# vrgamegirl19/comfyui-vrgamedevgirl

Hardware: NVIDIA H100
Metric: megapixels/sec (grain+LUT+colormatch+sharpen chain) at 4K (higher is better)
Workload: dtype f32

## Files before the change

### comfyui-vrgamedevgirl_b200/csrc/vrgdg_abi.cu

```cuda
#include "../../include/vrgdg_b200.h"
#include "vrgdg_kernels.cuh"
#include <cmath>
#include "vrgdg_adjust.cuh"
#include "vrgdg_resize.cuh"
#include "vrgdg_lanczos.cuh"
#include "vrgdg_temporal.cuh"
#include "vrgdg_histmatch.cuh"
#include <atomic>
#include <stdarg.h>
#include <stdio.h>
#include <stdlib.h>
#include <string.h>

namespace vrgdg {
static std::atomic<int64_t> g_launches{0};
void count_launch() { g_launches.fetch_add(1, std::memory_order_relaxed); }
}

using namespace vrgdg;

namespace {

thread_local char t_err[512] = "";
thread_local const char* t_tile_path = "none";
// ... 26 lines not shown
  }
  if (cached_major != 9 || cached_minor != 0)
    return fail(VRGDG_E_UNSUPPORTED, "libvrgdg_b200 holds sm_90a code only; device %d has compute capability %d.%d", dev, cached_major,
                cached_minor);
  ctx.stream = reinterpret_cast<cudaStream_t>(stream);
  ctx.sms = cached_sms;
  return VRGDG_OK;
}

int check_frames(const void* in, const void* out, int B, int H, int W, int dtype, const char* who) {
  if (!dtype_ok(dtype)) return fail(VRGDG_E_INVALID, "%s: unknown dtype %d", who, dtype);
  if (B < 0 || H < 0 || W < 0) return fail(VRGDG_E_INVALID, "%s: negative shape [%d,%d,%d]", who, B, H, W);
  if ((int64_t)H * W >= (int64_t)1 << 31) return fail(VRGDG_E_UNSUPPORTED, "%s: frame of %d x %d pixels exceeds 2^31", who, H, W);
  if ((int64_t)B * H * W == 0) return VRGDG_OK;
  if (!in || !out) return fail(VRGDG_E_INVALID, "%s: null frame pointer", who);
  size_t es = elem_size(dtype);
  if ((reinterpret_cast<uintptr_t>(in) % es) || (reinterpret_cast<uintptr_t>(out) % es))
    return fail(VRGDG_E_ALIGN, "%s: frame pointer not aligned to its element size", who);
  return VRGDG_OK;
}

#define DISPATCH_DTYPE(dtype, CALL)                                        \
  ((dtype) == VRGDG_F32 ? CALL(float) : ((dtype) == VRGDG_F16 ? CALL(__half) : ((dtype) == VRGDG_BF16 ? CALL(__nv_bfloat16) : CALL(uint8_t))))

typedef CUresult (*encode_fn_t)(CUtensorMap*, CUtensorMapDataType, cuuint32_t, void*, const cuuint64_t*,
                                const cuuint64_t*, const cuuint32_t*, const cuuint32_t*, CUtensorMapInterleave,
                                CUtensorMapSwizzle, CUtensorMapL2promotion, CUtensorMapFloatOOBfill);

encode_fn_t get_encode() {
  static encode_fn_t fn = []() -> encode_fn_t {
    void* p = nullptr;
    cudaDriverEntryPointQueryResult qr;
    if (cudaGetDriverEntryPoint("cuTensorMapEncodeTiled", &p, cudaEnableDefault, &qr) != cudaSuccess ||
        qr != cudaDriverEntryPointSuccess)
      return nullptr;
    return reinterpret_cast<encode_fn_t>(p);
  }();
  return fn;
}

bool build_tmap(CUtensorMap* map, const void* in, int B, int H, int RW, int dtype, int box_x, int box_y) {
  const size_t es = elem_size(dtype);
  if (getenv("VRGDG_NO_TMA")) return false;
  if ((reinterpret_cast<uintptr_t>(in) & 15u) || ((size_t)RW * es) % 16 != 0) return false;
  if (RW < box_x || H < box_y) return false;
  encode_fn_t enc = get_encode();
  if (!enc) return false;
  CUtensorMapDataType dt = dtype == VRGDG_F32 ? CU_TENSOR_MAP_DATA_TYPE_FLOAT32
                         : dtype == VRGDG_F16 ? CU_TENSOR_MAP_DATA_TYPE_FLOAT16
                         : dtype == VRGDG_BF16 ? CU_TENSOR_MAP_DATA_TYPE_BFLOAT16 : CU_TENSOR_MAP_DATA_TYPE_UINT8;
  cuuint64_t dims[3] = {(cuuint64_t)RW, (cuuint64_t)H, (cuuint64_t)B};
  cuuint64_t strides[2] = {(cuuint64_t)RW * es, (cuuint64_t)RW * es * (cuuint64_t)H};
  cuuint32_t box[3] = {(cuuint32_t)box_x, (cuuint32_t)box_y, 1u};
  cuuint32_t estr[3] = {1u, 1u, 1u};
  CUresult r = enc(map, dt, 3, const_cast<void*>(in), dims, strides, box, estr, CU_TENSOR_MAP_INTERLEAVE_NONE,
                   CU_TENSOR_MAP_SWIZZLE_NONE, CU_TENSOR_MAP_L2_PROMOTION_L2_128B, CU_TENSOR_MAP_FLOAT_OOB_FILL_NONE);
  return r == CUDA_SUCCESS;
}

size_t lut_cells_floats(int S) { return (size_t)S * S * S * LUT_CELL_FLOATS; }

void fill_lut(LutParams& L, const float* lut, int S, const float* dmin, const float* dspan, float blend, float omb) {
  L.lut = lut; L.S = S; L.smax = (float)(S - 1);
  L.lutp = lut + lut_cells_floats(S);
  for (int i = 0; i < 3; ++i) { L.dmin[i] = dmin[i]; L.dspan[i] = dspan[i]; }
  L.blend = blend; L.one_minus_blend = omb;
  L.unit_domain = (dmin[0] == 0.f && dmin[1] == 0.f && dmin[2] == 0.f && dspan[0] == 1.f && dspan[1] == 1.f && dspan[2] == 1.f) ? 1 : 0;
}

void zero_point(PointParams& P, int B, int H, int W) {
  memset(&P, 0, sizeof(P));
  P.B = B; P.H = H; P.W = W; P.hw = (int64_t)H * W;
}

int run_tile(const void* in, void* out, int B, int H, int W, int dtype, TileParams& Q, int mask, bool exact, const LaunchCtx& ctx) {
  if (in == out) return fail(VRGDG_E_INVALID, "tile kernels cannot run in place (in == out)");
  Q.B = B; Q.H = H; Q.W = W; Q.RW = 3 * W;
  int bx = 0, by = 0;
#define GEO(T) (tile_geometry<T>(H, Q.RW, Q.tiles_x, Q.tiles_y, bx, by), 0)
  (void)DISPATCH_DTYPE(dtype, GEO);
#undef GEO
  Q.total_tiles = (int64_t)B * Q.tiles_x * Q.tiles_y;
  if (Q.total_tiles >= ((int64_t)1 << 31)) return fail(VRGDG_E_UNSUPPORTED, "batch of %d frames has too many tiles for one launch; split it", B);
  CUtensorMap map;
  bool tma = build_tmap(&map, in, B, H, Q.RW, dtype, bx, by);
  Q.use_tma = tma ? 1 : 0;
  const size_t es = elem_size(dtype);
  Q.vec_store = (((size_t)Q.RW * es) % 16 == 0 && (reinterpret_cast<uintptr_t>(out) & 15u) == 0) ? 1 : 0;
  t_tile_path = tma ? "tma" : "generic";
#define TL(T) launch_tile<T>(tma ? &map : nullptr, in, out, Q, mask, exact, ctx)
  cudaError_t e = DISPATCH_DTYPE(dtype, TL);
#undef TL
  if (e != cudaSuccess) return fail_cuda(e, "k_tile launch");
  return VRGDG_OK;
}

int check_lut(const float* lut, int S, const float* dmin, const float* dspan, const char* who) {
  if (!lut || !dmin || !dspan) return fail(VRGDG_E_INVALID, "%s: null LUT / domain pointer", who);
  if (S < 2 || S > 256) return fail(VRGDG_E_INVALID, "%s: LUT size %d outside [2,256]", who, S);
  if (reinterpret_cast<uintptr_t>(lut) & 31u) return fail(VRGDG_E_ALIGN, "%s: packed LUT must be 32-byte aligned", who);
  return VRGDG_OK;
}

}

extern "C" {

int vrgdg_version(void) { return VRGDG_ABI_VERSION; }
const char* vrgdg_last_error(void) { return t_err; }
int64_t vrgdg_launch_count(void) { return g_launches.load(); }
const char* vrgdg_last_tile_path(void) { return t_tile_path; }

int vrgdg_device_info(int* sm_count, int* cc_major, int* cc_minor) {
  int dev = 0;
  cudaError_t e = cudaGetDevice(&dev);
  if (e != cudaSuccess) return fail_cuda(e, "cudaGetDevice");
  int v = 0;
  if (sm_count) { if ((e = cudaDeviceGetAttribute(&v, cudaDevAttrMultiProcessorCount, dev)) != cudaSuccess) return fail_cuda(e, "attr"); *sm_count = v; }
  if (cc_major) { if ((e = cudaDeviceGetAttribute(&v, cudaDevAttrComputeCapabilityMajor, dev)) != cudaSuccess) return fail_cuda(e, "attr"); *cc_major = v; }
  if (cc_minor) { if ((e = cudaDeviceGetAttribute(&v, cudaDevAttrComputeCapabilityMinor, dev)) != cudaSuccess) return fail_cuda(e, "attr"); *cc_minor = v; }
  return VRGDG_OK;
}

int64_t vrgdg_lut3d_packed_bytes(int lut_size) {
  if (lut_size < 2 || lut_size > 256) return 0;
  return (int64_t)lut_cells_floats(lut_size) * 2 * 4;
}

int vrgdg_lut3d_pack(const float* lut, float* packed, int lut_size, void* stream) {
  if (!lut || !packed) return fail(VRGDG_E_INVALID, "vrgdg_lut3d_pack: null pointer");
  if (lut_size < 2 || lut_size > 256) return fail(VRGDG_E_INVALID, "vrgdg_lut3d_pack: LUT size %d outside [2,256]", lut_size);
  if (reinterpret_cast<uintptr_t>(packed) & 31u) return fail(VRGDG_E_ALIGN, "vrgdg_lut3d_pack: packed buffer must be 32-byte aligned");
  LaunchCtx ctx;
  int rc = get_ctx(stream, ctx);
  if (rc) return rc;
  const int n = lut_size * lut_size * lut_size;
  k_lut_pack<<<(n + 255) / 256, 256, 0, ctx.stream>>>(lut, packed, lut_size);
  count_launch();
  k_lutp_pack<<<(n + 255) / 256, 256, 0, ctx.stream>>>(lut, packed + lut_cells_floats(lut_size), lut_size);
  count_launch();
  cudaError_t e = cudaGetLastError();
  if (e != cudaSuccess) return fail_cuda(e, "vrgdg_lut3d_pack");
  return VRGDG_OK;
}

int vrgdg_lut3d_apply(const void* in, void* out, int64_t npix, int channels, int dtype, const float* lut, int lut_size,
                      const float* dmin_host, const float* dspan_host, float blend, float one_minus_blend, void* stream) {
  if (!dtype_ok(dtype)) return fail(VRGDG_E_INVALID, "vrgdg_lut3d_apply: unknown dtype %d", dtype);
  if (channels != 3 && channels != 4) return fail(VRGDG_E_INVALID, "vrgdg_lut3d_apply: channels must be 3 or 4, got %d", channels);
  if (npix < 0) return fail(VRGDG_E_INVALID, "vrgdg_lut3d_apply: negative pixel count");
  if (!(blend > 0.0f) || blend > 1.0f) return fail(VRGDG_E_INVALID, "vrgdg_lut3d_apply: blend %g outside (0,1]", blend);
  int rc = check_lut(lut, lut_size, dmin_host, dspan_host, "vrgdg_lut3d_apply");
  if (rc) return rc;
  if (npix == 0) return VRGDG_OK;
  if (!in || !out) return fail(VRGDG_E_INVALID, "vrgdg_lut3d_apply: null frame pointer");
  LaunchCtx ctx;
  if ((rc = get_ctx(stream, ctx))) return rc;
  LutParams L;
  fill_lut(L, lut, lut_size, dmin_host, dspan_host, blend, one_minus_blend);
  cudaError_t e;
  if (channels == 4 && dtype == VRGDG_U8BGR) return fail(VRGDG_E_UNSUPPORTED, "vrgdg_lut3d_apply: 4-channel uint8 frames are not supported");
  if (channels == 4) {
#define LR(T) launch_lut_rgba<T>(in, out, npix, L, ctx)
    e = DISPATCH_DTYPE(dtype, LR);
#undef LR
  } else {
    const int64_t chunk = (int64_t)1 << 30;
    e = cudaSuccess;
    for (int64_t p0 = 0; p0 < npix && e == cudaSuccess; p0 += chunk) {
      int64_t n = npix - p0 < chunk ? npix - p0 : chunk;
      PointParams P;
      zero_point(P, 1, 1, (int)n);
      P.lut = L;
// ... 670 lines not shown
```

### comfyui-vrgamedevgirl_b200/csrc/vrgdg_inst.cuh

```cuda
#pragma once
#include "vrgdg_kernels.cuh"
#include <algorithm>
#include "vrgdg_adjust.cuh"
#include "vrgdg_resize.cuh"
#include "vrgdg_temporal.cuh"
#include "vrgdg_histmatch.cuh"
#include <string.h>
#include <stdlib.h>

namespace vrgdg {

static inline bool aligned16(const void* p) { return (reinterpret_cast<uintptr_t>(p) & 15u) == 0; }

template <typename K>
static int occupancy_of(K kernel, int threads, size_t smem) {
  int occ = 0;
  if (cudaOccupancyMaxActiveBlocksPerMultiprocessor(&occ, kernel, threads, smem) != cudaSuccess || occ < 1) occ = 1;
  return occ;
}

template <typename T, int MASK, bool EXACT, bool VEC>
static cudaError_t launch_point_k(const void* in, void* out, const PointParams& P, const LaunchCtx& ctx) {
  constexpr int PX = VEC ? (int)(3 * sizeof(typename Io<T>::word_t) / (3 * sizeof(T))) : 1;
  const int64_t groups = (P.hw + PX - 1) / PX;
  const int bpf = (int)((groups + 255) / 256);
  const int64_t total = (int64_t)bpf * P.B;
  if (total == 0) return cudaSuccess;
  auto kern = k_point<T, MASK, EXACT, VEC>;
  if (MASK & ST_LUT) cudaFuncSetAttribute(kern, cudaFuncAttributePreferredSharedMemoryCarveout, 0);
  static int occ = occupancy_of(kern, 256, 0);
  const int64_t cap = (int64_t)ctx.sms * occ * 4;
  const int grid = (int)std::min<int64_t>(total, cap);
  kern<<<grid, 256, 0, ctx.stream>>>(reinterpret_cast<const T*>(in), reinterpret_cast<T*>(out), P, bpf, total);
  count_launch();
  return cudaGetLastError();
}

template <typename T, int MASK, bool EXACT>
static cudaError_t launch_point_v(const void* in, void* out, const PointParams& P, const LaunchCtx& ctx) {
  typedef typename Io<T>::word_t word_t;
  constexpr int PX = (int)(3 * sizeof(word_t) / (3 * sizeof(T)));
  auto ok = [](const void* p) { return (reinterpret_cast<uintptr_t>(p) & (sizeof(word_t) - 1)) == 0; };
  bool vec = (P.hw % PX == 0) && (P.W % PX == 0) && ok(in) && ok(out) &&
             (!(MASK & ST_GRAIN) || P.ext_noise == nullptr || aligned16(P.ext_noise));
  if (vec) return launch_point_k<T, MASK, EXACT, true>(in, out, P, ctx);
  return launch_point_k<T, MASK, EXACT, false>(in, out, P, ctx);
}

template <typename T>
cudaError_t launch_point(const void* in, void* out, const PointParams& P, int mask, bool exact, const LaunchCtx& ctx) {
#define VRGDG_PT(M)                                                                    \
  case M:                                                                              \
    if constexpr (((M) & ST_GRAIN) != 0) {                                             \
      if (!exact) return launch_point_v<T, M, false>(in, out, P, ctx);                 \
    }                                                                                  \
    return launch_point_v<T, M, true>(in, out, P, ctx);
  switch (mask) {
    VRGDG_PT(1) VRGDG_PT(2) VRGDG_PT(3) VRGDG_PT(4) VRGDG_PT(5) VRGDG_PT(6) VRGDG_PT(7)
    case ST_CMF:
      if constexpr (sizeof(T) == 4) return launch_point_v<T, ST_CMF, true>(in, out, P, ctx);
      return cudaErrorInvalidValue;
    case ST_CMF | ST_LUT:
      if constexpr (sizeof(T) == 4) {
        if (!exact) return launch_point_v<T, ST_CMF | ST_LUT, false>(in, out, P, ctx);
        return launch_point_v<T, ST_CMF | ST_LUT, true>(in, out, P, ctx);
      }
      return cudaErrorInvalidValue;
    default: return cudaErrorInvalidValue;
  }
#undef VRGDG_PT
}

template <typename T>
cudaError_t launch_lut_rgba(const void* in, void* out, int64_t npix, const LutParams& L, const LaunchCtx& ctx) {
  if (npix == 0) return cudaSuccess;
  const int grid = (int)std::min<int64_t>((npix + 255) / 256, (int64_t)ctx.sms * 32);
  k_lut_rgba<T><<<grid, 256, 0, ctx.stream>>>(reinterpret_cast<const T*>(in), reinterpret_cast<T*>(out), npix, L);
  count_launch();
  return cudaGetLastError();
}

template <typename T>
void tile_geometry(int H, int RW, int& tiles_x, int& tiles_y, int& box_x, int& box_y) {
  using C = TileCfg<T, 0>;
  tiles_x = (RW + C::TXE - 1) / C::TXE;
  tiles_y = (H + C::TY - 1) / C::TY;
  box_x = C::BX;
  box_y = C::ROWS;
}

template <typename T, int MASK, bool EXACT>
static cudaError_t launch_tile_k(const CUtensorMap* tmap, const void* in, void* out, TileParams& Q, const LaunchCtx& ctx) {
  auto kern = k_tile<T, MASK, EXACT>;
  constexpr size_t smem = tile_smem_bytes<T, MASK>();
  cudaError_t attr = cudaFuncSetAttribute(kern, cudaFuncAttributeMaxDynamicSharedMemorySize, (int)smem);
  if (attr != cudaSuccess) return attr;
  constexpr int NT = TileCfg<T, MASK>::THREADS;
  if (MASK & ST_LUT) cudaFuncSetAttribute(kern, cudaFuncAttributePreferredSharedMemoryCarveout, (int)((smem + 1024) * TileCfg<T, MASK>::MINB * 100 / (228 * 1024)) + 1);
  static int occ = occupancy_of(kern, NT, smem);
  if (Q.total_tiles == 0) return cudaSuccess;
  int grid = (int)std::min<int64_t>(Q.total_tiles, (int64_t)ctx.sms * occ);
  if (Q.grid_limit > 0 && grid > Q.grid_limit) grid = Q.grid_limit;
  CUtensorMap dummy;
  if (!tmap) { memset(&dummy, 0, sizeof(dummy)); tmap = &dummy; }
  kern<<<grid, NT, smem, ctx.stream>>>(*tmap, reinterpret_cast<const T*>(in), reinterpret_cast<T*>(out), Q);
  count_launch();
  return cudaGetLastError();
}

template <typename T>
cudaError_t launch_tile(const CUtensorMap* tmap, const void* in, void* out, TileParams& Q, int mask, bool exact,
                        const LaunchCtx& ctx) {
#define VRGDG_TL(M)                                                                        \
  case M:                                                                                  \
    if constexpr (((M) & ST_GRAIN) != 0) {                                                 \
      if (!exact) return launch_tile_k<T, M, false>(tmap, in, out, Q, ctx);                \
    }                                                                                      \
    return launch_tile_k<T, M, true>(tmap, in, out, Q, ctx);
  switch (mask) {
    VRGDG_TL(0) VRGDG_TL(1) VRGDG_TL(2) VRGDG_TL(3) VRGDG_TL(4) VRGDG_TL(5) VRGDG_TL(6) VRGDG_TL(7)
    VRGDG_TL(8)
    case ST_CMF:
      if constexpr (sizeof(T) == 4) return launch_tile_k<T, ST_CMF, true>(tmap, in, out, Q, ctx);
      return cudaErrorInvalidValue;
    case ST_CMF | ST_LUT:
      if constexpr (sizeof(T) == 4) {
        if (!exact) return launch_tile_k<T, ST_CMF | ST_LUT, false>(tmap, in, out, Q, ctx);
        return launch_tile_k<T, ST_CMF | ST_LUT, true>(tmap, in, out, Q, ctx);
      }
      return cudaErrorInvalidValue;
    default: return cudaErrorInvalidValue;
  }
#undef VRGDG_TL
}

template <typename T, bool GRAIN, bool VEC, int NT>
static cudaError_t launch_moments_k(const T* src, const PointParams& P, int row0, int rows, double* partials, float* fplanes, const LaunchCtx& ctx) {
  auto kern = k_lab_moments<T, GRAIN, VEC, NT>;
  if (NT == MOMENT_UNIT) {
    cudaFuncSetAttribute(kern, cudaFuncAttributePreferredSharedMemoryCarveout, 64);
  }
  dim3 grid(MOMENT_BLOCKS / (NT / MOMENT_UNIT), P.B);
  kern<<<grid, NT, 0, ctx.stream>>>(src, P, row0, rows, partials, fplanes);
  count_launch();
  return cudaGetLastError();
}

template <typename T>
cudaError_t launch_moments(const void* in, const PointParams& P, bool grain, int row0, int rows, double* sums,
                           double* partials, const LaunchCtx& ctx, float* fplanes, bool small_blocks) {
  if (P.B == 0) return cudaSuccess;
  typedef typename Io<T>::word_t word_t;
  constexpr int PX = (int)(sizeof(word_t) / sizeof(T));
  const bool vec = (P.W % PX == 0) && ((reinterpret_cast<uintptr_t>(in) & (sizeof(word_t) - 1)) == 0);
  if (fplanes && !(vec && sizeof(T) == 4 && aligned16(fplanes))) return cudaErrorInvalidValue;
  const T* src = reinterpret_cast<const T*>(in);
  cudaError_t e;
  if (small_blocks && vec && grain) e = launch_moments_k<T, true, true, MOMENT_UNIT>(src, P, row0, rows, partials, fplanes, ctx);
  else if (small_blocks && vec) e = launch_moments_k<T, false, true, MOMENT_UNIT>(src, P, row0, rows, partials, fplanes, ctx);
  else if (grain && vec) e = launch_moments_k<T, true, true, 256>(src, P, row0, rows, partials, fplanes, ctx);
  else if (grain) e = launch_moments_k<T, true, false, 256>(src, P, row0, rows, partials, fplanes, ctx);
  else if (vec) e = launch_moments_k<T, false, true, 256>(src, P, row0, rows, partials, fplanes, ctx);
  else e = launch_moments_k<T, false, false, 256>(src, P, row0, rows, partials, fplanes, ctx);
  if (e != cudaSuccess) return e;
  k_moments_final<<<P.B, 32, 0, ctx.stream>>>(partials, MOMENT_BLOCKS, (double)rows * (double)P.W, sums);
  count_launch();
  return cudaGetLastError();
}

template <typename T>
cudaError_t launch_u8_in(const uint8_t* in, void* out, int64_t npix, const LaunchCtx& ctx) {
  if (npix == 0) return cudaSuccess;
  const int grid = (int)std::min<int64_t>((npix + 255) / 256, (int64_t)ctx.sms * 32);
  k_u8bgr_to_rgb<T><<<grid, 256, 0, ctx.stream>>>(in, reinterpret_cast<T*>(out), npix);
  count_launch();
  return cudaGetLastError();
}
template <typename T>
cudaError_t launch_u8_out(const void* in, uint8_t* out, int64_t npix, const LaunchCtx& ctx) {
  if (npix == 0) return cudaSuccess;
  const int grid = (int)std::min<int64_t>((npix + 255) / 256, (int64_t)ctx.sms * 32);
  k_rgb_to_u8bgr<T><<<grid, 256, 0, ctx.stream>>>(reinterpret_cast<const T*>(in), out, npix);
  count_launch();
  return cudaGetLastError();
}

#define VRGDG_INSTANTIATE(T)                                                                                              \
  template cudaError_t launch_point<T>(const void*, void*, const PointParams&, int, bool, const LaunchCtx&);              \
  template cudaError_t launch_lut_rgba<T>(const void*, void*, int64_t, const LutParams&, const LaunchCtx&);               \
  template cudaError_t launch_tile<T>(const CUtensorMap*, const void*, void*, TileParams&, int, bool, const LaunchCtx&);  \
  template cudaError_t launch_moments<T>(const void*, const PointParams&, bool, int, int, double*, double*, const LaunchCtx&, float*, bool); \
  template cudaError_t launch_adjust<T>(const void*, void*, const AdjustParams&, int, float*, float*, const LaunchCtx&);              \
  template cudaError_t launch_resize<T>(const void*, void*, const ResizeParams&, const LaunchCtx&);                       \
  template cudaError_t launch_blend<T>(const void*, const void*, void*, int64_t, float, float, const LaunchCtx&);         \
  template cudaError_t launch_temporal<T>(const void*, void*, const TemporalParams&, const LaunchCtx&);                   \
  template cudaError_t launch_hist_counts<T>(const void*, int, int, int, int, int, uint32_t*, const LaunchCtx&);          \
  template cudaError_t launch_histmatch_apply<T>(const void*, void*, int, int64_t, const float2*, float, float, const LaunchCtx&); \
  template void tile_geometry<T>(int, int, int&, int&, int&, int&);

#define VRGDG_INSTANTIATE_CODECS(T)                                                                                       \
  template cudaError_t launch_u8_in<T>(const uint8_t*, void*, int64_t, const LaunchCtx&);                                 \
  template cudaError_t launch_u8_out<T>(const void*, uint8_t*, int64_t, const LaunchCtx&);

}
```

### comfyui-vrgamedevgirl_b200/csrc/vrgdg_kernels.cuh

```cuda
#pragma once
#include <cuda.h>
#include <cuda_runtime.h>
#include <cuda_fp16.h>
#include <cuda_bf16.h>
#include <stdint.h>
#include "vrgdg_math.cuh"

namespace vrgdg {

enum {
  ST_GRAIN = 1, ST_CM = 2, ST_LUT = 4,
  ST_POST = 8,
  ST_CMF = 16,
  ST_PRE = ST_GRAIN | ST_CM | ST_LUT | ST_CMF
};

template <typename T> struct Elem;
template <> struct Elem<float> {
  static __device__ __forceinline__ float ld(float v) { return v; }
  static __device__ __forceinline__ float st(float v) { return v; }
};
template <> struct Elem<__half> {
  static __device__ __forceinline__ float ld(__half v) { return __half2float(v); }
  static __device__ __forceinline__ __half st(float v) { return __float2half_rn(v); }
// ... 211 lines not shown
__device__ __forceinline__ void fence_mbar_init() { asm volatile("fence.mbarrier_init.release.cluster;" ::: "memory"); }
__device__ __forceinline__ void fence_proxy_async() { asm volatile("fence.proxy.async.shared::cta;" ::: "memory"); }
__device__ __forceinline__ void mbar_arrive_expect_tx(uint64_t* bar, uint32_t bytes) {
  asm volatile("mbarrier.arrive.expect_tx.shared::cta.b64 _, [%0], %1;" ::"r"(smem_u32(bar)), "r"(bytes) : "memory");
}
__device__ __forceinline__ bool mbar_try_wait(uint64_t* bar, uint32_t parity) {
  uint32_t ok;
  asm volatile(
      "{\n .reg .pred p;\n mbarrier.try_wait.parity.shared::cta.b64 p, [%1], %2;\n selp.u32 %0, 1, 0, p;\n}"
      : "=r"(ok) : "r"(smem_u32(bar)), "r"(parity) : "memory");
  return ok != 0;
}
__device__ __forceinline__ uint64_t globaltimer_ns() {
  uint64_t t;
  asm volatile("mov.u64 %0, %%globaltimer;" : "=l"(t));
  return t;
}
__device__ __forceinline__ void mbar_wait(uint64_t* bar, uint32_t parity) {
  if (mbar_try_wait(bar, parity)) return;
#pragma unroll 1
  for (int i = 0; i < 64; ++i)
    if (mbar_try_wait(bar, parity)) return;
  const uint64_t t0 = globaltimer_ns();
  uint32_t ns = 32;
  while (!mbar_try_wait(bar, parity)) {
    __nanosleep(ns);
    if (ns < 1024) ns <<= 1;
    if (globaltimer_ns() - t0 > 20000000000ull) __trap();
  }
}
__device__ __forceinline__ void tma_load_3d(void* smem_dst, const CUtensorMap* tmap, int c0, int c1, int c2,
                                            uint64_t* bar) {
  asm volatile(
      "cp.async.bulk.tensor.3d.shared::cluster.global.tile.mbarrier::complete_tx::bytes [%0], [%1, {%2, %3, %4}], [%5];"
      ::"r"(smem_u32(smem_dst)), "l"((uint64_t)tmap), "r"(c0), "r"(c1), "r"(c2), "r"(smem_u32(bar))
      : "memory");
}

struct TileParams {
  int B, H, W, RW;
  int tiles_x, tiles_y;
  int64_t total_tiles;
  PointParams P;
  int op;
  float strength;
  int border;
  int post_enabled;
  float pI, ps, poms;
  uint64_t pseed;
  int64_t pframe0;
  int pseed_mode;
  GrainKey pkey;
  int exact_stencil;
  int use_tma;
  int vec_store;
  int grid_limit;
};

template <typename T, int MASK> struct TileCfg {
  static constexpr bool HEAVY = (MASK & ST_LUT) != 0;
  static constexpr bool WORK = (sizeof(T) == 1) || (((MASK & ST_PRE) != 0) && (sizeof(T) != 4));
  static constexpr bool GPLANE = (MASK & ST_POST) != 0;
  static constexpr int VEC = WORK ? 4 : 16 / (int)sizeof(T);
  static constexpr int BX = 256;
  static constexpr int PADL = 16 / (int)sizeof(T);
  static constexpr int TXE = sizeof(T) == 1 ? 192 : 240;
#ifndef VRGDG_TILE_ROWS
#define VRGDG_TILE_ROWS 32
#endif
  static constexpr int TY = VRGDG_TILE_ROWS;
  static constexpr int ROWS = TY + 2;
#ifndef VRGDG_HEAVY_THREADS
#define VRGDG_HEAVY_THREADS 256
#endif
  static constexpr int THREADS = HEAVY ? VRGDG_HEAVY_THREADS : 256;
#ifndef VRGDG_HEAVY_LB
#define VRGDG_HEAVY_LB 352
#endif
  static constexpr int LB_THREADS = (HEAVY && sizeof(T) == 4 && VRGDG_HEAVY_LB > THREADS) ? VRGDG_HEAVY_LB : THREADS;
#ifndef VRGDG_HEAVY_MINB
#define VRGDG_HEAVY_MINB 2
#endif
#ifndef VRGDG_HEAVY_NS
#define VRGDG_HEAVY_NS (WORK ? 1 : 2)
#endif
#ifndef VRGDG_LIGHT_MINB
#define VRGDG_LIGHT_MINB 2
#endif
#ifndef VRGDG_LIGHT_NS
#define VRGDG_LIGHT_NS 3
#endif
  static constexpr bool SLIM = (MASK == 0) && (sizeof(T) == 2);
  static constexpr int MINB = HEAVY ? VRGDG_HEAVY_MINB : (SLIM ? 4 : VRGDG_LIGHT_MINB);
  static constexpr int COLS = TXE / VEC;
  static constexpr int RG = (THREADS / COLS) >= 8 ? 8 : 4;
  static constexpr int RPT = TY / RG;
  static constexpr int PPR = TXE / 3 + 2;
  static constexpr int PAIRS = PPR / 2 + 1;
  static constexpr int NS = HEAVY ? VRGDG_HEAVY_NS : ((GPLANE || SLIM) ? 2 : VRGDG_LIGHT_NS);
  static constexpr int STAGE_BYTES = ROWS * BX * (int)sizeof(T);
  static_assert(PADL + TXE + 3 <= BX, "box too narrow");
  static_assert(TY % RG == 0 && COLS * RG <= THREADS, "thread mapping");
};

template <typename T, int MASK>
constexpr size_t tile_smem_bytes() {
  using C = TileCfg<T, MASK>;
  size_t s = (size_t)C::NS * C::STAGE_BYTES;
  if (C::WORK) s += (size_t)C::ROWS * C::BX * 4;
  if (C::GPLANE) s += (size_t)C::ROWS * C::BX * 4;
  return s + 64  + 128 ;
}

template <typename E, typename CFG>
__device__ __forceinline__ void fix_border(E* tile, int y0, int x0e, int H, int RW) {
  constexpr int BX = CFG::BX, ROWS = CFG::ROWS, PADL = CFG::PADL, TY = CFG::TY, TXE = CFG::TXE;
  const int vr = H - y0;
  const int ve = RW - x0e;
  const bool top = (y0 == 0), bot = (vr <= TY), left = (x0e == 0), right = (ve <= TXE);
  if (!(top || bot || left || right)) return;
  if (top || bot) {
    for (int c = threadIdx.x; c < BX; c += blockDim.x) {
      if (top) tile[c] = tile[BX + c];
      if (bot) tile[(vr + 1) * BX + c] = tile[vr * BX + c];
    }
  }
  __syncthreads();
  if (left || right) {
    for (int i = threadIdx.x; i < ROWS * 3; i += blockDim.x) {
      int r = i / 3, c = i - r * 3;
      E* row = tile + r * BX;
      if (left) row[PADL - 3 + c] = row[PADL + c];
      if (right) row[PADL + ve + c] = row[PADL + ve - 3 + c];
    }
  }
  __syncthreads();
}

__device__ __forceinline__ uint4 lds128(const void* p) {
  uint4 v;
  asm volatile("ld.shared.v4.u32 {%0, %1, %2, %3}, [%4];" : "=r"(v.x), "=r"(v.y), "=r"(v.z), "=r"(v.w) : "r"(smem_u32(p)) : "memory");
  return v;
}

template <typename E, int VEC>
__device__ __forceinline__ void load_window(const E* rowp , float* w) {
  if (sizeof(E) == 4) {
    constexpr int NV = (VEC + 8) / 4;
    float tmp[NV * 4];
    const float* p = reinterpret_cast<const float*>(rowp) - 4;
#pragma unroll
    for (int i = 0; i < NV; ++i) {
      const uint4 q = lds128(p + 4 * i);
      tmp[4 * i] = __uint_as_float(q.x); tmp[4 * i + 1] = __uint_as_float(q.y);
      tmp[4 * i + 2] = __uint_as_float(q.z); tmp[4 * i + 3] = __uint_as_float(q.w);
    }
#pragma unroll
    for (int i = 0; i < VEC + 6; ++i) w[i] = tmp[i + 1];
  } else {
    union { uint4 q[3]; E e[24]; } u;
    u.q[0] = lds128(rowp - 8); u.q[1] = lds128(rowp); u.q[2] = lds128(rowp + 8);
#pragma unroll
    for (int i = 0; i < VEC + 6; ++i) w[i] = Elem<E>::ld(u.e[i + 5]);
  }
}

template <int VEC, bool BGR>
__device__ __forceinline__ void post_grain_elems(const TileParams& Q, const GrainFrame& gf, int ge0, int y, float* o) {
  const int pfirst = ge0 / 3, plast = (ge0 + VEC - 1) / 3;
  constexpr int NPR = (VEC + 1) / 3 + 1;
#pragma unroll
  for (int q = 0; q < NPR; ++q) {
    const int pair = (pfirst >> 1) + q;
    if (pair * 2 > plast) break;
    float z[6];
    grain_pair_normals(grain_pair_bits(Q.pkey, gf, (uint32_t)pair, (uint32_t)y), z);
    const float gy0 = Q.poms * z[1], gy1 = Q.poms * z[4];
    const float g0 = fmaf(2.0f * Q.ps, z[0], gy0), g1 = fmaf(Q.ps, z[1], gy0), g2 = fmaf(3.0f * Q.ps, z[2], gy0);
    const float g3 = fmaf(2.0f * Q.ps, z[3], gy1), g4 = fmaf(Q.ps, z[4], gy1), g5 = fmaf(3.0f * Q.ps, z[5], gy1);
#pragma unroll
    for (int e = 0; e < VEC; ++e) {
      const int idx = ge0 + e - pair * 6;
      if (idx >= 0 && idx < 6) {
        const float lo = (idx == 0) ? (BGR ? g2 : g0) : ((idx == 1) ? g1 : (BGR ? g0 : g2));
        const float hi = (idx == 3) ? (BGR ? g5 : g3) : ((idx == 4) ? g4 : (BGR ? g3 : g5));
        const float gv = (idx < 3) ? lo : hi;
        o[e] = clamp01(fmaf(Q.pI, gv, o[e]));
      }
    }
  }
}

template <typename T, int VEC>
__device__ __forceinline__ void store_elems(T* __restrict__ out, const TileParams& Q, int frame, int y, int ge0, const float* o) {
// ... 52 lines not shown
    for (int j = 0; j < C::RPT; ++j) {
      load_row(rbase + j + 2, wr);
      const int y = y0 + rbase + j;
      float o[VEC];
#pragma unroll
      for (int e = 0; e < VEC; ++e) {
        const float h2 = (wr[e] + wr[e + 3]) + wr[e + 6];
        const float blur = ((h0[e] + h1[e]) + h2) * 0.1111111111111111f;
        o[e] = clamp01(fmaf(Q.strength, c1[e] - blur, c1[e]));
        h0[e] = h1[e]; h1[e] = h2; c1[e] = wr[e + 3];
      }
      if constexpr (C::GPLANE) {
        const float4* gp = reinterpret_cast<const float4*>(gplane + (rbase + j + 1) * BX + PADL + f0);
#pragma unroll
        for (int q = 0; q < VEC / 4; ++q) {
          const float4 gv = gp[q];
          o[4 * q] = clamp01(fmaf(Q.pI, gv.x, o[4 * q])); o[4 * q + 1] = clamp01(fmaf(Q.pI, gv.y, o[4 * q + 1]));
          o[4 * q + 2] = clamp01(fmaf(Q.pI, gv.z, o[4 * q + 2])); o[4 * q + 3] = clamp01(fmaf(Q.pI, gv.w, o[4 * q + 3]));
        }
      } else if ((MASK & ST_PRE) != 0 && Q.post_enabled) post_grain_elems<VEC, Io<T>::BGR>(Q, pgf, ge0, y, o);
      store_elems<T, VEC>(out, Q, frame, y, ge0, o);
    }
  } else {
    float w[3][WN];
    load_row(rbase, w[0]);
    load_row(rbase + 1, w[1]);
#pragma unroll
    for (int j = 0; j < C::RPT; ++j) {
      load_row(rbase + j + 2, w[2]);
      const int y = y0 + rbase + j;
      float o[VEC];
#pragma unroll
      for (int e = 0; e < VEC; ++e) {
        float n[9] = {w[0][e], w[0][e + 3], w[0][e + 6], w[1][e], w[1][e + 3], w[1][e + 6],
                      w[2][e], w[2][e + 3], w[2][e + 6]};
        o[e] = XS ? stencil_epilogue_exact(OP, n, Q.strength) : stencil_epilogue(OP, n, Q.strength);
      }
      if constexpr (C::GPLANE) {
        const float4* gp = reinterpret_cast<const float4*>(gplane + (rbase + j + 1) * BX + PADL + f0);
#pragma unroll
        for (int q = 0; q < VEC / 4; ++q) {
          const float4 gv = gp[q];
          o[4 * q] = clamp01(fmaf(Q.pI, gv.x, o[4 * q])); o[4 * q + 1] = clamp01(fmaf(Q.pI, gv.y, o[4 * q + 1]));
          o[4 * q + 2] = clamp01(fmaf(Q.pI, gv.z, o[4 * q + 2])); o[4 * q + 3] = clamp01(fmaf(Q.pI, gv.w, o[4 * q + 3]));
        }
      } else if ((MASK & ST_PRE) != 0 && Q.post_enabled) post_grain_elems<VEC, Io<T>::BGR>(Q, pgf, ge0, y, o);
      store_elems<T, VEC>(out, Q, frame, y, ge0, o);
#pragma unroll
      for (int i = 0; i < WN; ++i) { w[0][i] = w[1][i]; w[1][i] = w[2][i]; }
    }
  }
}

template <typename T>
__device__ __forceinline__ void pair_load6(const T* p, bool word0, float* e) {
  if (sizeof(T) == 4) {
    const float2* q = reinterpret_cast<const float2*>(p);
    if (word0) { float2 v = q[0]; e[0] = v.x; e[1] = v.y; }
    float2 v1 = q[1], v2 = q[2];
    e[2] = v1.x; e[3] = v1.y; e[4] = v2.x; e[5] = v2.y;
  } else if (sizeof(T) == 2) {
    const uint32_t* q = reinterpret_cast<const uint32_t*>(p);
    union { uint32_t u[3]; T h[6]; } w;
    w.u[0] = word0 ? q[0] : 0u; w.u[1] = q[1]; w.u[2] = q[2];
#pragma unroll
    for (int i = 0; i < 6; ++i) e[i] = Elem<T>::ld(w.h[i]);
  } else {
    const uint16_t* q = reinterpret_cast<const uint16_t*>(p);
    union { uint16_t u[3]; T h[6]; } w;
    w.u[0] = word0 ? q[0] : (uint16_t)0; w.u[1] = q[1]; w.u[2] = q[2];
#pragma unroll
    for (int i = 0; i < 6; ++i) e[i] = Elem<T>::ld(w.h[i]);
  }
}
__device__ __forceinline__ void pair_store6(float* p, bool word0, const float* e) {
  float2* q = reinterpret_cast<float2*>(p);
  if (word0) q[0] = make_float2(e[0], e[1]);
  q[1] = make_float2(e[2], e[3]);
  q[2] = make_float2(e[4], e[5]);
}

template <typename T, int MASK, bool EXACT>
__global__ void __launch_bounds__((TileCfg<T, MASK>::LB_THREADS), (TileCfg<T, MASK>::MINB))
k_tile(const __grid_constant__ CUtensorMap tmap, const T* __restrict__ in, T* __restrict__ out, TileParams Q) {
  using C = TileCfg<T, MASK>;
  constexpr int NT = C::THREADS;
  constexpr int VEC = C::VEC, BX = C::BX, PADL = C::PADL, TXE = C::TXE, TY = C::TY, ROWS = C::ROWS;
  constexpr int NS = C::NS;
  constexpr bool WORK = C::WORK;

  extern __shared__ uint8_t smem_raw[];
  const uint32_t smem_a = smem_u32(smem_raw);
  uint8_t* base = smem_raw + (((smem_a + 127u) & ~127u) - smem_a);
  T* stage0 = reinterpret_cast<T*>(base);
  constexpr bool GPLANE = C::GPLANE;
  float* work = reinterpret_cast<float*>(base + (size_t)NS * C::STAGE_BYTES);
  float* gplane = reinterpret_cast<float*>(base + (size_t)NS * C::STAGE_BYTES + (WORK ? ROWS * BX * 4 : 0));
  uint64_t* bars = reinterpret_cast<uint64_t*>(base + (size_t)NS * C::STAGE_BYTES + (WORK ? ROWS * BX * 4 : 0) + (GPLANE ? ROWS * BX * 4 : 0));

  const int tid = threadIdx.x;
  const uint32_t first = blockIdx.x, stride = gridDim.x, total = (uint32_t)Q.total_tiles;
  const uint32_t n_my = (total > first) ? (total - first + stride - 1) / stride : 0;
  const uint32_t tiles_per_frame = (uint32_t)(Q.tiles_x * Q.tiles_y);
  const bool tma = Q.use_tma != 0;

  if (tma && tid == 0) {
#pragma unroll
    for (int s = 0; s < NS; ++s) mbar_init(&bars[s], 1);
    fence_mbar_init();
    fence_proxy_async();
  }
  __syncthreads();

  auto tile_coords = [&](uint32_t k, int& frame, int& y0, int& x0e) {
    const uint32_t t = first + k * stride;
    const uint32_t f = t / tiles_per_frame;
    const uint32_t rem = t - f * tiles_per_frame;
    const uint32_t ty = rem / (uint32_t)Q.tiles_x;
    frame = (int)f;
    y0 = (int)ty * TY;
    x0e = (int)(rem - ty * (uint32_t)Q.tiles_x) * TXE;
  };
  auto issue = [&](uint32_t k) {
    int frame, y0, x0e;
    tile_coords(k, frame, y0, x0e);
    int s = (int)(k % NS);
    mbar_arrive_expect_tx(&bars[s], (uint32_t)C::STAGE_BYTES);
    tma_load_3d(reinterpret_cast<uint8_t*>(stage0) + (size_t)s * C::STAGE_BYTES, &tmap, x0e - PADL, y0 - 1, frame, &bars[s]);
  };

#ifndef VRGDG_EARLY_REFILL
#define VRGDG_EARLY_REFILL 1
#endif
  constexpr bool EARLY = WORK && (VRGDG_EARLY_REFILL != 0);
  constexpr bool LATE1 = !EARLY && NS == 1;
  constexpr uint32_t AHEAD = EARLY ? NS : (LATE1 ? 1 : NS - 1);
  if (tma && tid == 0) {
    for (uint32_t k = 0; k < AHEAD && k < n_my; ++k) issue(k);
  }

  for (uint32_t k = 0; k < n_my; ++k) {
    int frame, y0, x0e;
    tile_coords(k, frame, y0, x0e);
    const int s = tma ? (int)(k % NS) : 0;
    T* raw = reinterpret_cast<T*>(reinterpret_cast<uint8_t*>(stage0) + (size_t)s * C::STAGE_BYTES);

    if (tma) {
      if (!EARLY && !LATE1 && tid == 0 && k + NS - 1 < n_my) {
        fence_proxy_async();
        issue(k + NS - 1);
      }
      mbar_wait(&bars[s], (uint32_t)((k / NS) & 1));
    } else {
      const T* fbase = in + (int64_t)frame * Q.H * Q.RW;
      for (int i = tid; i < ROWS * BX; i += NT) {
        int r = i / BX, c = i - r * BX;
        int y = y0 - 1 + r, x = x0e - PADL + c;
        T v = Elem<T>::st(0.0f);
        if (y >= 0 && y < Q.H && x >= 0 && x < Q.RW) v = fbase[(int64_t)y * Q.RW + x];
        raw[i] = v;
      }
      __syncthreads();
    }

    if ((MASK & ST_PRE) != 0 || WORK || GPLANE) {
      const PointParams& P = Q.P;
      constexpr bool GRAIN = (MASK & ST_GRAIN) != 0;
      constexpr bool BGR = Io<T>::BGR;
      typedef typename Io<T>::noise_t noise_t;
      const GrainFrame gf = grain_frame(P.seed, P.frame0, frame, P.seed_mode);
      CmFold cmf = {};
      if (MASK & (ST_CM | ST_CMF)) cmf = cm_fold(P.cm_params + (int64_t)frame * 12, P.cm_t, P.cm_omt);
      const bool has_ext = GRAIN && (P.ext_noise != nullptr);
      const GrainFrame pgf = grain_frame(Q.pseed, Q.pframe0, frame, Q.pseed_mode);
      const int pair0 = x0e / 6 - 1;
      for (int i = tid; i < ROWS * C::PAIRS; i += NT) {
        const int r = i / C::PAIRS, kx = i - r * C::PAIRS;
        const int y = y0 - 1 + r, pair = pair0 + kx;
        const int pxa = pair * 2;
        const int so = r * BX + PADL - 6 + 6 * kx;
        const bool rowin = (y >= 0 && y < Q.H);
        const bool need_a = (kx > 0), need_b = (kx < C::PAIRS - 1);
        const bool in_a = need_a && rowin && pxa >= 0 && pxa < Q.W;
        const bool in_b = need_b && rowin && pxa + 1 >= 0 && pxa + 1 < Q.W;
        if (GPLANE) {
          float gz[6] = {0.f, 0.f, 0.f, 0.f, 0.f, 0.f};
          if (rowin && pair >= 0 && pxa < Q.W) {
            float z[6];
            grain_pair_normals(grain_pair_bits(Q.pkey, pgf, (uint32_t)pair, (uint32_t)y), z);
            const float gy0 = Q.poms * z[1], gy1 = Q.poms * z[4];
            const float r0 = fmaf(2.0f * Q.ps, z[0], gy0), g0 = fmaf(Q.ps, z[1], gy0), b0 = fmaf(3.0f * Q.ps, z[2], gy0);
            const float r1 = fmaf(2.0f * Q.ps, z[3], gy1), g1 = fmaf(Q.ps, z[4], gy1), b1 = fmaf(3.0f * Q.ps, z[5], gy1);
            gz[0] = BGR ? b0 : r0; gz[1] = g0; gz[2] = BGR ? r0 : b0;
            gz[3] = BGR ? b1 : r1; gz[4] = g1; gz[5] = BGR ? r1 : b1;
          }
          pair_store6(gplane + so, kx > 0, gz);
        }
        if ((MASK & ST_PRE) == 0 && !WORK) continue;
        float e[6] = {0.f, 0.f, 0.f, 0.f, 0.f, 0.f};
        if (in_a | in_b) {
          pair_load6<T>(raw + so, kx > 0, e);
          float z[6] = {0.f, 0.f, 0.f, 0.f, 0.f, 0.f};
          if (GRAIN) {
            if (has_ext) {
              const noise_t* ns = reinterpret_cast<const noise_t*>(P.ext_noise) + ((int64_t)frame * P.hw + (int64_t)y * Q.W + pxa) * 3;
              if (in_a) { z[0] = noise_ld<noise_t>(ns[0]); z[1] = noise_ld<noise_t>(ns[1]); z[2] = noise_ld<noise_t>(ns[2]); }
              if (in_b) { z[3] = noise_ld<noise_t>(ns[3]); z[4] = noise_ld<noise_t>(ns[4]); z[5] = noise_ld<noise_t>(ns[5]); }
            } else {
              grain_pair_normals(grain_pair_bits(P.gkey, gf, (uint32_t)pair, (uint32_t)y), z);
            }
          }
          float p[6] = {e[BGR ? 2 : 0], e[1], e[BGR ? 0 : 2], e[BGR ? 5 : 3], e[4], e[BGR ? 3 : 5]};
          process_pair<MASK, EXACT>(P, cmf, z, p);
          if (in_a) { e[BGR ? 2 : 0] = p[0]; e[1] = p[1]; e[BGR ? 0 : 2] = p[2]; } else if (WORK) { e[0] = 0.f; e[1] = 0.f; e[2] = 0.f; }
          if (in_b) { e[BGR ? 5 : 3] = p[3]; e[4] = p[4]; e[BGR ? 3 : 5] = p[5]; } else if (WORK) { e[3] = 0.f; e[4] = 0.f; e[5] = 0.f; }
        }
        if constexpr (WORK) {
          pair_store6(work + so, kx > 0, e);
        } else {
          if (in_a | in_b) pair_store6(reinterpret_cast<float*>(raw) + so, kx > 0, e);
        }
      }
      __syncthreads();
      if (EARLY && tma && tid == 0 && k + NS < n_my) {
        fence_proxy_async();
        issue(k + NS);
      }
    }

    if (Q.border == 0) {
      if constexpr (WORK) fix_border<float, C>(work, y0, x0e, Q.H, Q.RW);
      else fix_border<T, C>(raw, y0, x0e, Q.H, Q.RW);
    }

    {
      const float* wt = WORK ? work : nullptr;
      if (Q.exact_stencil) {
        switch (Q.op) {
          case 1: stencil_rows<T, 1, MASK, true>(raw, wt, gplane, out, Q, frame, y0, x0e); break;
          case 2: stencil_rows<T, 2, MASK, true>(raw, wt, gplane, out, Q, frame, y0, x0e); break;
          case 3: stencil_rows<T, 3, MASK, false>(raw, wt, gplane, out, Q, frame, y0, x0e); break;
          case 4: stencil_rows<T, 4, MASK, true>(raw, wt, gplane, out, Q, frame, y0, x0e); break;
          case 5: stencil_rows<T, 5, MASK, false>(raw, wt, gplane, out, Q, frame, y0, x0e); break;
          default: stencil_rows<T, 0, MASK, false>(raw, wt, gplane, out, Q, frame, y0, x0e); break;
        }
      } else {
        switch (Q.op) {
          case 1: stencil_rows<T, 1, MASK, false>(raw, wt, gplane, out, Q, frame, y0, x0e); break;
          case 2: stencil_rows<T, 2, MASK, false>(raw, wt, gplane, out, Q, frame, y0, x0e); break;
          case 3: stencil_rows<T, 3, MASK, false>(raw, wt, gplane, out, Q, frame, y0, x0e); break;
          case 4: stencil_rows<T, 4, MASK, false>(raw, wt, gplane, out, Q, frame, y0, x0e); break;
          case 5: stencil_rows<T, 5, MASK, false>(raw, wt, gplane, out, Q, frame, y0, x0e); break;
          default: stencil_rows<T, 0, MASK, false>(raw, wt, gplane, out, Q, frame, y0, x0e); break;
        }
      }
    }
    if (tma) fence_proxy_async();
    __syncthreads();
    if (LATE1 && tma && tid == 0 && k + 1 < n_my) issue(k + 1);
  }
}

constexpr int MOMENT_BLOCKS = 592;
constexpr int MOMENT_UNIT = 128;

__device__ __forceinline__ double warp_sum(double v) {
#pragma unroll
  for (int o = 16; o > 0; o >>= 1) v += __shfl_xor_sync(0xffffffffu, v, o);
  return v;
}

__device__ __forceinline__ void moments_add(float& r, float& g, float& b, float* s1, float* s2) {
  float fx, fy, fz;
  rgb_to_fxyz(r, g, b, fx, fy, fz);
  r = fx; g = fy; b = fz;
  const float u1 = fx - fy, u2 = fy - fz;
  s1[0] += fy; s1[1] += u1; s1[2] += u2;
  s2[0] = fmaf(fy, fy, s2[0]); s2[1] = fmaf(u1, u1, s2[1]); s2[2] = fmaf(u2, u2, s2[2]);
}

#ifndef VRGDG_MOMENT_SMALL_MINB
#define VRGDG_MOMENT_SMALL_MINB 10
#endif
template <int NT> struct MomentLaunch { static constexpr int MINB = (NT == MOMENT_UNIT) ? VRGDG_MOMENT_SMALL_MINB : 4; };
template <typename T, bool GRAIN, bool VEC, int NT>
__global__ void __launch_bounds__(NT, (MomentLaunch<NT>::MINB))
k_lab_moments(const T* __restrict__ in, PointParams P, int row0, int rows, double* __restrict__ partials, float* __restrict__ fplanes) {
  static_assert(NT % MOMENT_UNIT == 0, "whole reduction units per block");
  constexpr int UPB = NT / MOMENT_UNIT;
  const int unit = blockIdx.x * UPB + (threadIdx.x / MOMENT_UNIT), ut = threadIdx.x % MOMENT_UNIT;
  typedef typename Io<T>::word_t word_t;
  typedef typename Io<T>::noise_t noise_t;
  constexpr bool BGR = Io<T>::BGR;
  constexpr int PX = VEC ? (int)(sizeof(word_t) / sizeof(T)) : 1;
  constexpr int NE = PX * 3;
  const int frame = blockIdx.y;
  const int64_t pbeg = (int64_t)row0 * P.W, n = (int64_t)rows * P.W;
  const T* fbase = in + (int64_t)frame * P.hw * 3;
  const GrainFrame gf = grain_frame(P.seed, P.frame0, frame, P.seed_mode);
  const bool has_ext = GRAIN && (P.ext_noise != nullptr);
  const CmFold nocm = {};
  double acc[6] = {0, 0, 0, 0, 0, 0};
  const int64_t groups = (n + PX - 1) / PX;
  for (int64_t gi = (int64_t)unit * MOMENT_UNIT + ut; gi < groups; gi += (int64_t)MOMENT_BLOCKS * MOMENT_UNIT) {
    const int64_t pif = pbeg + gi * PX;
    float v[NE], nz[NE];
    union { word_t q[3]; T e[NE]; } u;
    if (VEC) {
      const word_t* src = reinterpret_cast<const word_t*>(fbase + pif * 3);
      u.q[0] = __ldg(src); u.q[1] = __ldg(src + 1); u.q[2] = __ldg(src + 2);
    } else {
#pragma unroll
      for (int i = 0; i < NE; ++i) u.e[i] = fbase[pif * 3 + i];
    }
#pragma unroll
    for (int j = 0; j < PX; ++j) {
#pragma unroll
      for (int c = 0; c < 3; ++c) v[3 * j + c] = Elem<T>::ld(u.e[3 * j + (BGR ? 2 - c : c)]);
    }
    if (GRAIN) {
      const uint32_t y = (uint32_t)pif / (uint32_t)P.W, x = (uint32_t)pif - y * (uint32_t)P.W;
      if (has_ext) {
        const noise_t* ns = reinterpret_cast<const noise_t*>(P.ext_noise) + ((int64_t)frame * P.hw + pif) * 3;
#pragma unroll
        for (int i = 0; i < NE; ++i) nz[i] = noise_ld<noise_t>(ns[i]);
#pragma unroll
        for (int j = 0; j < PX; ++j)
          process_pixel<ST_GRAIN, true>(P, nocm, nz[3 * j], nz[3 * j + 1], nz[3 * j + 2], v[3 * j], v[3 * j + 1], v[3 * j + 2]);
      } else if (VEC) {
#pragma unroll
        for (int j = 0; j < PX; j += 2) {
          float z[6];
          grain_pair_normals(grain_pair_bits(P.gkey, gf, (x >> 1) + (uint32_t)(j >> 1), y), z);
          process_pixel<ST_GRAIN, false>(P, nocm, z[0], z[1], z[2], v[3 * j], v[3 * j + 1], v[3 * j + 2]);
          process_pixel<ST_GRAIN, false>(P, nocm, z[3], z[4], z[5], v[3 * j + 3], v[3 * j + 4], v[3 * j + 5]);
        }
      } else {
        float zr, zg, zb;
        grain_pixel_normals(P.gkey, gf, x, y, zr, zg, zb);
// ... 148 lines not shown
```

Measured before the change: 36630.

## Walk tiles in vertical strips and carry halo rows between consecutive tiles

For pipelines with a pre stage, each block now processes a contiguous run of tiles down a vertical column strip. It copies the two bottom halo rows of the previous tile (after pre-processing) into the top of the next stage buffer, so only TY new rows are loaded through a second TMA descriptor and the pre-stage work (grain, LUT) is not repeated on halo rows. Blocks may be paired across adjacent strips, the heavy-config stage count drops to 1, and the carveout is computed by a shared helper that is also applied to the moments kernel. The gains come at the cost of extra syncs, a serial dependency between tiles within a block, and less pipelining depth.

Result: no change. 36350 (median of 6 runs) (-0.8%).

```diff
diff --git a/comfyui-vrgamedevgirl_b200/csrc/vrgdg_abi.cu b/comfyui-vrgamedevgirl_b200/csrc/vrgdg_abi.cu
--- a/comfyui-vrgamedevgirl_b200/csrc/vrgdg_abi.cu
+++ b/comfyui-vrgamedevgirl_b200/csrc/vrgdg_abi.cu
@@ -132,13 +132,13 @@
 #undef GEO
   Q.total_tiles = (int64_t)B * Q.tiles_x * Q.tiles_y;
   if (Q.total_tiles >= ((int64_t)1 << 31)) return fail(VRGDG_E_UNSUPPORTED, "batch of %d frames has too many tiles for one launch; split it", B);
-  CUtensorMap map;
-  bool tma = build_tmap(&map, in, B, H, Q.RW, dtype, bx, by);
+  CUtensorMap map[2];
+  bool tma = build_tmap(&map[0], in, B, H, Q.RW, dtype, bx, by) && build_tmap(&map[1], in, B, H, Q.RW, dtype, bx, by - 2);
   Q.use_tma = tma ? 1 : 0;
   const size_t es = elem_size(dtype);
   Q.vec_store = (((size_t)Q.RW * es) % 16 == 0 && (reinterpret_cast<uintptr_t>(out) & 15u) == 0) ? 1 : 0;
   t_tile_path = tma ? "tma" : "generic";
-#define TL(T) launch_tile<T>(tma ? &map : nullptr, in, out, Q, mask, exact, ctx)
+#define TL(T) launch_tile<T>(tma ? map : nullptr, in, out, Q, mask, exact, ctx)
   cudaError_t e = DISPATCH_DTYPE(dtype, TL);
 #undef TL
   if (e != cudaSuccess) return fail_cuda(e, "k_tile launch");
diff --git a/comfyui-vrgamedevgirl_b200/csrc/vrgdg_inst.cuh b/comfyui-vrgamedevgirl_b200/csrc/vrgdg_inst.cuh
--- a/comfyui-vrgamedevgirl_b200/csrc/vrgdg_inst.cuh
+++ b/comfyui-vrgamedevgirl_b200/csrc/vrgdg_inst.cuh
@@ -96,14 +96,14 @@
   cudaError_t attr = cudaFuncSetAttribute(kern, cudaFuncAttributeMaxDynamicSharedMemorySize, (int)smem);
   if (attr != cudaSuccess) return attr;
   constexpr int NT = TileCfg<T, MASK>::THREADS;
-  if (MASK & ST_LUT) cudaFuncSetAttribute(kern, cudaFuncAttributePreferredSharedMemoryCarveout, (int)((smem + 1024) * TileCfg<T, MASK>::MINB * 100 / (228 * 1024)) + 1);
+  if (MASK & ST_LUT) cudaFuncSetAttribute(kern, cudaFuncAttributePreferredSharedMemoryCarveout, tile_carveout<T, MASK>());
   static int occ = occupancy_of(kern, NT, smem);
   if (Q.total_tiles == 0) return cudaSuccess;
   int grid = (int)std::min<int64_t>(Q.total_tiles, (int64_t)ctx.sms * occ);
   if (Q.grid_limit > 0 && grid > Q.grid_limit) grid = Q.grid_limit;
-  CUtensorMap dummy;
-  if (!tmap) { memset(&dummy, 0, sizeof(dummy)); tmap = &dummy; }
-  kern<<<grid, NT, smem, ctx.stream>>>(*tmap, reinterpret_cast<const T*>(in), reinterpret_cast<T*>(out), Q);
+  CUtensorMap dummy[2];
+  if (!tmap) { memset(dummy, 0, sizeof(dummy)); tmap = dummy; }
+  kern<<<grid, NT, smem, ctx.stream>>>(tmap[0], tmap[1], reinterpret_cast<const T*>(in), reinterpret_cast<T*>(out), Q);
   count_launch();
   return cudaGetLastError();
 }
@@ -138,7 +138,7 @@
 static cudaError_t launch_moments_k(const T* src, const PointParams& P, int row0, int rows, double* partials, float* fplanes, const LaunchCtx& ctx) {
   auto kern = k_lab_moments<T, GRAIN, VEC, NT>;
   if (NT == MOMENT_UNIT) {
-    cudaFuncSetAttribute(kern, cudaFuncAttributePreferredSharedMemoryCarveout, 64);
+    cudaFuncSetAttribute(kern, cudaFuncAttributePreferredSharedMemoryCarveout, tile_carveout<float, ST_CMF | ST_LUT>());
   }
   dim3 grid(MOMENT_BLOCKS / (NT / MOMENT_UNIT), P.B);
   kern<<<grid, NT, 0, ctx.stream>>>(src, P, row0, rows, partials, fplanes);
diff --git a/comfyui-vrgamedevgirl_b200/csrc/vrgdg_kernels.cuh b/comfyui-vrgamedevgirl_b200/csrc/vrgdg_kernels.cuh
--- a/comfyui-vrgamedevgirl_b200/csrc/vrgdg_kernels.cuh
+++ b/comfyui-vrgamedevgirl_b200/csrc/vrgdg_kernels.cuh
@@ -317,7 +317,7 @@
 #define VRGDG_HEAVY_MINB 2
 #endif
 #ifndef VRGDG_HEAVY_NS
-#define VRGDG_HEAVY_NS (WORK ? 1 : 2)
+#define VRGDG_HEAVY_NS 1
 #endif
 #ifndef VRGDG_LIGHT_MINB
 #define VRGDG_LIGHT_MINB 2
@@ -345,6 +345,11 @@
   if (C::WORK) s += (size_t)C::ROWS * C::BX * 4;
   if (C::GPLANE) s += (size_t)C::ROWS * C::BX * 4;
   return s + 64  + 128 ;
+}
+
+template <typename T, int MASK>
+constexpr int tile_carveout() {
+  return (int)((tile_smem_bytes<T, MASK>() + 1024) * TileCfg<T, MASK>::MINB * 100 / (228 * 1024)) + 1;
 }
 
 template <typename E, typename CFG>
@@ -563,12 +568,14 @@
 
 template <typename T, int MASK, bool EXACT>
 __global__ void __launch_bounds__((TileCfg<T, MASK>::LB_THREADS), (TileCfg<T, MASK>::MINB))
-k_tile(const __grid_constant__ CUtensorMap tmap, const T* __restrict__ in, T* __restrict__ out, TileParams Q) {
+k_tile(const __grid_constant__ CUtensorMap tmap, const __grid_constant__ CUtensorMap tmap_rows, const T* __restrict__ in,
+       T* __restrict__ out, TileParams Q) {
   using C = TileCfg<T, MASK>;
   constexpr int NT = C::THREADS;
   constexpr int VEC = C::VEC, BX = C::BX, PADL = C::PADL, TXE = C::TXE, TY = C::TY, ROWS = C::ROWS;
   constexpr int NS = C::NS;
   constexpr bool WORK = C::WORK;
+  constexpr bool CARRY = (MASK & ST_PRE) != 0;
 
   extern __shared__ uint8_t smem_raw[];
   const uint32_t smem_a = smem_u32(smem_raw);
@@ -580,9 +587,17 @@
   uint64_t* bars = reinterpret_cast<uint64_t*>(base + (size_t)NS * C::STAGE_BYTES + (WORK ? ROWS * BX * 4 : 0) + (GPLANE ? ROWS * BX * 4 : 0));
 
   const int tid = threadIdx.x;
-  const uint32_t first = blockIdx.x, stride = gridDim.x, total = (uint32_t)Q.total_tiles;
-  const uint32_t n_my = (total > first) ? (total - first + stride - 1) / stride : 0;
-  const uint32_t tiles_per_frame = (uint32_t)(Q.tiles_x * Q.tiles_y);
+  const uint32_t total = (uint32_t)Q.total_tiles;
+  const bool paired = CARRY && gridDim.x % 2 == 0 && Q.tiles_x % 2 == 0;
+  const uint32_t groups = paired ? gridDim.x / 2 : gridDim.x;
+  const uint32_t cg = blockIdx.x % groups, side = blockIdx.x / groups;
+  const uint32_t units = paired ? total / 2 : total;
+  const uint32_t strips = paired ? (uint32_t)Q.tiles_x / 2 : (uint32_t)Q.tiles_x;
+  const uint32_t first = CARRY ? (uint32_t)((uint64_t)cg * units / groups) : blockIdx.x;
+  const uint32_t stride = CARRY ? 1u : gridDim.x;
+  const uint32_t n_my = CARRY ? (uint32_t)((uint64_t)(cg + 1) * units / groups) - first
+                              : ((total > first) ? (total - first + stride - 1) / stride : 0);
+  const uint32_t tiles_per_frame = CARRY ? strips * (uint32_t)Q.tiles_y : (uint32_t)(Q.tiles_x * Q.tiles_y);
   const bool tma = Q.use_tma != 0;
 
   if (tma && tid == 0) {
@@ -597,17 +612,30 @@
     const uint32_t t = first + k * stride;
     const uint32_t f = t / tiles_per_frame;
     const uint32_t rem = t - f * tiles_per_frame;
-    const uint32_t ty = rem / (uint32_t)Q.tiles_x;
     frame = (int)f;
-    y0 = (int)ty * TY;
-    x0e = (int)(rem - ty * (uint32_t)Q.tiles_x) * TXE;
+    if (CARRY) {
+      const uint32_t sp = rem / (uint32_t)Q.tiles_y;
+      y0 = (int)(rem - sp * (uint32_t)Q.tiles_y) * TY;
+      x0e = (int)(paired ? 2 * sp + side : sp) * TXE;
+    } else {
+      const uint32_t ty = rem / (uint32_t)Q.tiles_x;
+      y0 = (int)ty * TY;
+      x0e = (int)(rem - ty * (uint32_t)Q.tiles_x) * TXE;
+    }
   };
+  auto carried = [&](uint32_t k, int y0) { return CARRY && k > 0 && y0 > 0; };
   auto issue = [&](uint32_t k) {
     int frame, y0, x0e;
     tile_coords(k, frame, y0, x0e);
     int s = (int)(k % NS);
-    mbar_arrive_expect_tx(&bars[s], (uint32_t)C::STAGE_BYTES);
-    tma_load_3d(reinterpret_cast<uint8_t*>(stage0) + (size_t)s * C::STAGE_BYTES, &tmap, x0e - PADL, y0 - 1, frame, &bars[s]);
+    uint8_t* dst = reinterpret_cast<uint8_t*>(stage0) + (size_t)s * C::STAGE_BYTES;
+    if (carried(k, y0)) {
+      mbar_arrive_expect_tx(&bars[s], (uint32_t)(TY * BX * sizeof(T)));
+      tma_load_3d(dst + 2 * BX * sizeof(T), &tmap_rows, x0e - PADL, y0 + 1, frame, &bars[s]);
+    } else {
+      mbar_arrive_expect_tx(&bars[s], (uint32_t)C::STAGE_BYTES);
+      tma_load_3d(dst, &tmap, x0e - PADL, y0 - 1, frame, &bars[s]);
+    }
   };
 
 #ifndef VRGDG_EARLY_REFILL
@@ -625,6 +653,7 @@
     tile_coords(k, frame, y0, x0e);
     const int s = tma ? (int)(k % NS) : 0;
     T* raw = reinterpret_cast<T*>(reinterpret_cast<uint8_t*>(stage0) + (size_t)s * C::STAGE_BYTES);
+    const int r0 = carried(k, y0) ? 2 : 0;
 
     if (tma) {
       if (!EARLY && !LATE1 && tid == 0 && k + NS - 1 < n_my) {
@@ -634,7 +663,7 @@
       mbar_wait(&bars[s], (uint32_t)((k / NS) & 1));
     } else {
       const T* fbase = in + (int64_t)frame * Q.H * Q.RW;
-      for (int i = tid; i < ROWS * BX; i += NT) {
+      for (int i = r0 * BX + tid; i < ROWS * BX; i += NT) {
         int r = i / BX, c = i - r * BX;
         int y = y0 - 1 + r, x = x0e - PADL + c;
         T v = Elem<T>::st(0.0f);
@@ -655,7 +684,7 @@
       const bool has_ext = GRAIN && (P.ext_noise != nullptr);
       const GrainFrame pgf = grain_frame(Q.pseed, Q.pframe0, frame, Q.pseed_mode);
       const int pair0 = x0e / 6 - 1;
-      for (int i = tid; i < ROWS * C::PAIRS; i += NT) {
+      for (int i = r0 * C::PAIRS + tid; i < ROWS * C::PAIRS; i += NT) {
         const int r = i / C::PAIRS, kx = i - r * C::PAIRS;
         const int y = y0 - 1 + r, pair = pair0 + kx;
         const int pxa = pair * 2;
@@ -736,6 +765,14 @@
         }
       }
     }
+    if (CARRY && k + 1 < n_my && y0 + TY < Q.H) {
+      const bool same = WORK || NS == 1 || !tma;
+      float* src = WORK ? work : reinterpret_cast<float*>(raw);
+      float* dst = same ? src : reinterpret_cast<float*>(reinterpret_cast<uint8_t*>(stage0) + (size_t)((k + 1) % NS) * C::STAGE_BYTES);
+      if (same) __syncthreads();
+      for (int i = tid; i < 2 * BX / 4; i += NT)
+        reinterpret_cast<float4*>(dst)[i] = reinterpret_cast<const float4*>(src + TY * BX)[i];
+    }
     if (tma) fence_proxy_async();
     __syncthreads();
     if (LATE1 && tma && tid == 0 && k + 1 < n_my) issue(k + 1);
```
